# td-kwj-zp2023/webgpu-msm-bls12-377

Hardware: AMD Instinct MI355X
Metric: ms per 2^20 BLS12-377 G1 MSM (lower is better)
Workload: dtype u32 (29-bit limbs, 64-bit accumulate)

## Files before the change

webgpu-msm-bls12-377_amd/csrc/kernels/convert.hpp:

```cpp
#pragma once
#include "../curves.hpp"

namespace msm377 {
namespace {


__global__ void __launch_bounds__(256) k_clear_words(uint32_t* __restrict__ a, uint32_t na, uint32_t* __restrict__ b, uint32_t nb) {
  for (uint32_t i = threadIdx.x; i < na; i += 256) a[i] = 0;
  for (uint32_t i = threadIdx.x; i < nb; i += 256) b[i] = 0;
}

template <class CV>
__global__ void __launch_bounds__(256) k_convert_bases(const uint32_t* __restrict__ raw, uint32_t* __restrict__ bases, uint64_t n, int* __restrict__ err) {
  uint64_t i = (uint64_t)blockIdx.x * 256 + threadIdx.x;
  if (i >= n) return;
  uint32_t w[CV::RAW_WORDS];
  load_words16(raw + i * CV::RAW_WORDS, w, CV::RAW_WORDS / 4);
  uint32_t o[CV::REC_WORDS];
  if (CV::convert(w, o)) atomicOr(err, ERR_TE_CONVERT);
  uint4* dst = reinterpret_cast<uint4*>(bases + i * CV::REC_WORDS);
#pragma unroll
  for (int k = 0; k < (int)CV::REC_WORDS / 4; k++) dst[k] = make_uint4(o[4 * k], o[4 * k + 1], o[4 * k + 2], o[4 * k + 3]);
}


__device__ __forceinline__ void put13(uint32_t* w, const Fp::El& e) {
#pragma unroll
  for (int j = 0; j < 13; j++) w[j] = e.l[j];
}
__device__ __forceinline__ Fp::El get13(const uint32_t* w) {
  Fp::El e;
#pragma unroll
  for (int j = 0; j < 13; j++) e.l[j] = w[j];
  return e;
}
struct AffWireSource {
  const uint32_t* raw;
  __device__ __forceinline__ bool load(uint64_t i, Fp::El& n1, Fp::El& n2, Fp::El& z) const {
    using K = G1Consts;
    uint32_t w[24];
    load_words16(raw + i * 24, w, 6);
    const Fp::El xr = Fp::from_words<12>(w), yr = Fp::from_words<12>(w + 12);
    const Fp::El u = Fp::add_lz(Fp::mul_lz(xr, Fp::from_const(K::TE_SR)), Fp::from_const(K::TE_S));
    const Fp::El v = Fp::mul_lz(yr, Fp::from_const(K::TE_SR));
    const Fp::El cu = Fp::csub(Fp::norm(Fp::add_lz(Fp::mul_lz(xr, Fp::from_const(K::TE_CSR)), Fp::from_const(K::TE_CS))), K::MOD);
    const Fp::El up = Fp::add_lz(u, Fp::one());
    z = Fp::mul_lz(up, v);
    n1 = Fp::mul_lz(up, cu);
    n2 = Fp::norm(Fp::add_kp_sub_sub2(z, K::KP4W3, Fp::zero(), v));
    return Te377::is_zero_mod_p(z);
  }
};
struct AffDoublingSource {
  const uint32_t* prev;
  uint32_t bits;
  __device__ __forceinline__ bool load(uint64_t i, Fp::El& n1, Fp::El& n2, Fp::El& z) const {
    Te377::Ext p = Te377::from_base_affine(TeAffBase::load_base(prev, (uint32_t)i), false);
    bool bad = false;
#pragma unroll 1
    for (uint32_t k = 0; k < bits; k++) {
      p = Te377::add(p, p);
      bad |= Te377::is_bad(p);
    }
    n1 = Fp::canon(p.x);
    n2 = Fp::canon(p.y);
    z = Fp::canon(p.z);
    return bad;
  }
};
template <class SRC>
__global__ void __launch_bounds__(AFF_THREADS, 4) k_affine_up(SRC src, uint64_t n, uint32_t* __restrict__ stash,
                                                              uint32_t* __restrict__ trees, uint32_t* __restrict__ block_prod, uint32_t* __restrict__ host_flag, uint32_t* __restrict__ dev_count,
                                                              int* __restrict__ err, uint32_t prio) {
  if (prio) __builtin_amdgcn_s_setprio(3);
  using K = G1Consts;
  __shared__ uint32_t tree[2 * AFF_THREADS][13];
  const uint32_t tid = threadIdx.x, blk = blockIdx.x;
  const uint64_t base = (uint64_t)blk * AFF_BLOCK_POINTS + tid;
  bool bad = false;
  Fp::El c = Fp::one();
#pragma unroll 1
  for (uint32_t j = 0; j < AFF_K; j++) {
    const uint64_t i = base + (uint64_t)j * AFF_THREADS;
    if (i >= n) break;
    Fp::El n1, n2, z;
    if (src.load(i, n1, n2, z)) {
      bad = true;
      z = Fp::one();
    }
    uint32_t o[AFF_STASH_WORDS];
    put13(o, n1);
    put13(o + 13, n2);
    put13(o + 26, z);
    put13(o + 39, c);
    uint4* dst = reinterpret_cast<uint4*>(stash) + ((size_t)blk * AFF_K + j) * (AFF_STASH_WORDS / 4) * AFF_THREADS + tid;
#pragma unroll
    for (int k = 0; k < (int)AFF_STASH_WORDS / 4; k++) dst[(size_t)k * AFF_THREADS] = make_uint4(o[4 * k], o[4 * k + 1], o[4 * k + 2], o[4 * k + 3]);
    c = Fp::mul_lz(c, z);
  }
  if (bad) atomicOr(err, ERR_TE_CONVERT);
  put13(tree[AFF_THREADS + tid], c);
  for (uint32_t size = AFF_THREADS / 2; size >= 1; size >>= 1) {
    __syncthreads();
    if (tid < size) put13(tree[size + tid], Fp::mul_lz(get13(tree[2 * (size + tid)]), get13(tree[2 * (size + tid) + 1])));
  }
  __syncthreads();
  uint32_t* out = trees + (size_t)blk * (2 * AFF_THREADS * 13);
  const uint32_t* flat = &tree[0][0];
  for (uint32_t k = tid; k < 2 * AFF_THREADS * 13; k += AFF_THREADS) out[k] = flat[k];
  if (tid == 0) {
    const Fp::El root = Fp::mul(get13(tree[1]), Fp::from_const(K::TO64));
    uint32_t w[12];
    Fp::to_words<12>(root, w);
#pragma unroll
    for (int j = 0; j < 12; j++) block_prod[(size_t)blk * 12 + j] = w[j];
    __threadfence_system();
    if (atomicAdd(dev_count, 1u) == gridDim.x - 1) {
      *dev_count = 0;
      __threadfence_system();
      *reinterpret_cast<volatile uint32_t*>(host_flag) = gridDim.x;
    }
  }
}

__global__ void __launch_bounds__(AFF_THREADS, 2) k_affine_down(uint64_t n, const uint32_t* __restrict__ stash, const uint32_t* __restrict__ trees,
                                                                const uint32_t* __restrict__ block_inv, uint32_t* __restrict__ bases, uint32_t prio) {
  if (prio) __builtin_amdgcn_s_setprio(3);
  __shared__ uint32_t tree[2 * AFF_THREADS][13];
  const uint32_t tid = threadIdx.x, blk = blockIdx.x;
  const uint32_t* in = trees + (size_t)blk * (2 * AFF_THREADS * 13);
  uint32_t* flat = &tree[0][0];
  for (uint32_t k = tid; k < 2 * AFF_THREADS * 13; k += AFF_THREADS) flat[k] = in[k];
  __syncthreads();
  if (tid == 0) {
    uint32_t w[12];
#pragma unroll
    for (int j = 0; j < 12; j++) w[j] = block_inv[(size_t)blk * 12 + j];
    put13(tree[1], Fp::from_words<12>(w));
  }
  for (uint32_t size = 1; size < AFF_THREADS; size <<= 1) {
    __syncthreads();
    if (tid < size) {
      const uint32_t k = size + tid;
      const Fp::El inv_k = get13(tree[k]), a = get13(tree[2 * k]), b = get13(tree[2 * k + 1]);
      put13(tree[2 * k], Fp::mul_lz(inv_k, b));
      put13(tree[2 * k + 1], Fp::mul_lz(inv_k, a));
    }
  }
  __syncthreads();
  Fp::El inv = get13(tree[AFF_THREADS + tid]);
  const uint64_t base = (uint64_t)blk * AFF_BLOCK_POINTS + tid;
#pragma unroll 1
  for (int j = (int)AFF_K - 1; j >= 0; j--) {
    const uint64_t i = base + (uint64_t)j * AFF_THREADS;
    if (i >= n) continue;
    uint32_t w[AFF_STASH_WORDS];
    {
      const uint4* src = reinterpret_cast<const uint4*>(stash) + ((size_t)blk * AFF_K + j) * (AFF_STASH_WORDS / 4) * AFF_THREADS + tid;
#pragma unroll
      for (int k = 0; k < (int)AFF_STASH_WORDS / 4; k++) {
        const uint4 v = src[(size_t)k * AFF_THREADS];
        w[4 * k + 0] = v.x;
        w[4 * k + 1] = v.y;
        w[4 * k + 2] = v.z;
        w[4 * k + 3] = v.w;
      }
    }
    const Fp::El zi = Fp::mul_lz(inv, get13(w + 39));
    inv = Fp::mul_lz(inv, get13(w + 26));
    const Fp::El x = Fp::mul(get13(w), zi), y = Fp::mul(get13(w + 13), zi);
    const Fp::El ymx = Fp::sub(y, x), ypx = Fp::add(y, x), kt = Fp::mul_lz(Fp::mul_lz(x, y), Fp::from_const(G1Consts::TE_2D));
    uint32_t o[TeAffBase::REC_WORDS];
    put13(o, ymx);
    put13(o + 13, ypx);
    put13(o + 26, kt);
    o[39] = 0;
    uint4* dst = reinterpret_cast<uint4*>(bases + i * TeAffBase::REC_WORDS);
#pragma unroll
    for (int k = 0; k < (int)TeAffBase::REC_WORDS / 4; k++) dst[k] = make_uint4(o[4 * k], o[4 * k + 1], o[4 * k + 2], o[4 * k + 3]);
  }
}


__global__ void __launch_bounds__(256) k_convert_bases_glv(const uint32_t* __restrict__ raw, uint32_t* __restrict__ bases, uint64_t n) {
  uint64_t i = (uint64_t)blockIdx.x * 256 + threadIdx.x;
  if (i >= n) return;
  uint32_t w[24];
  load_words16(raw + i * 24, w, 6);
  const Fp::El x = Fp::to_mont(Fp::from_words<12>(w));
  const Fp::El y = Fp::to_mont(Fp::from_words<12>(w + 12));
  const Fp::El bx = Fp::mul(x, Fp::from_const(G1Consts::BETA));
  constexpr uint32_t REC_WORDS = G1Dev::REC_WORDS;
  uint32_t o[REC_WORDS];
#pragma unroll
  for (int j = 0; j < 13; j++) {
    o[j] = x.l[j];
    o[13 + j] = y.l[j];
  }
#pragma unroll
  for (int j = 26; j < 32; j++) o[j] = 0;
  uint4* dst = reinterpret_cast<uint4*>(bases + i * REC_WORDS);
#pragma unroll
  for (int k = 0; k < 8; k++) dst[k] = make_uint4(o[4 * k], o[4 * k + 1], o[4 * k + 2], o[4 * k + 3]);
#pragma unroll
  for (int j = 0; j < 13; j++) o[j] = bx.l[j];
  dst = reinterpret_cast<uint4*>(bases + (n + i) * REC_WORDS);
#pragma unroll
  for (int k = 0; k < 8; k++) dst[k] = make_uint4(o[4 * k], o[4 * k + 1], o[4 * k + 2], o[4 * k + 3]);
}


}
}
```

Measured before the change: 2.369.

## Prefetch stash rows and coalesce affine base stores through LDS in affine_down

Restructures the backward loop of k_affine_down so the next stash row is requested into registers before the current row's field arithmetic runs, hiding global load latency. Output records are staged in padded shared memory and then written to global memory in a block-wide coalesced pattern instead of each thread writing its own 160-byte record with strided uint4 stores. The tree buffer is aliased onto the new LDS staging array. This adds two barriers per row and more live registers for the prefetch buffer, which may reduce occupancy.

```diff
diff --git a/webgpu-msm-bls12-377_amd/csrc/kernels/convert.hpp b/webgpu-msm-bls12-377_amd/csrc/kernels/convert.hpp
--- a/webgpu-msm-bls12-377_amd/csrc/kernels/convert.hpp
+++ b/webgpu-msm-bls12-377_amd/csrc/kernels/convert.hpp
@@ -123,10 +123,20 @@
   }
 }
 
+constexpr uint32_t AFF_REC_PIECES = TeAffBase::REC_WORDS / 4, AFF_REC_PITCH = AFF_REC_PIECES + 1;
+constexpr uint32_t AFF_REC_LDS = AFF_THREADS * AFF_REC_PITCH;
+static_assert(AFF_REC_LDS >= 2 * AFF_THREADS * 13 / 4, "the tree fits the buffer");
+__device__ __forceinline__ uint32_t affine_rows(uint64_t first, uint64_t n) {
+  if (first >= n) return 0;
+  const uint64_t r = (n - first + AFF_THREADS - 1) / AFF_THREADS;
+  return r < AFF_K ? (uint32_t)r : AFF_K;
+}
+
 __global__ void __launch_bounds__(AFF_THREADS, 2) k_affine_down(uint64_t n, const uint32_t* __restrict__ stash, const uint32_t* __restrict__ trees,
                                                                 const uint32_t* __restrict__ block_inv, uint32_t* __restrict__ bases, uint32_t prio) {
   if (prio) __builtin_amdgcn_s_setprio(3);
-  __shared__ uint32_t tree[2 * AFF_THREADS][13];
+  __shared__ uint4 lds[AFF_REC_LDS];
+  uint32_t(*tree)[13] = reinterpret_cast<uint32_t(*)[13]>(lds);
   const uint32_t tid = threadIdx.x, blk = blockIdx.x;
   const uint32_t* in = trees + (size_t)blk * (2 * AFF_THREADS * 13);
   uint32_t* flat = &tree[0][0];
@@ -149,35 +159,52 @@
   }
   __syncthreads();
   Fp::El inv = get13(tree[AFF_THREADS + tid]);
-  const uint64_t base = (uint64_t)blk * AFF_BLOCK_POINTS + tid;
+  __syncthreads();
+  const uint64_t first = (uint64_t)blk * AFF_BLOCK_POINTS, base = first + tid;
+  const uint32_t rows = affine_rows(first, n);
+  constexpr uint32_t STASH_PIECES = AFF_STASH_WORDS / 4;
+  uint4 next[STASH_PIECES];
+  auto request = [&](uint32_t j) {
+    const uint4* src = reinterpret_cast<const uint4*>(stash) + ((size_t)blk * AFF_K + j) * STASH_PIECES * AFF_THREADS + tid;
+    const bool mine = base + (uint64_t)j * AFF_THREADS < n;
+#pragma unroll
+    for (uint32_t k = 0; k < STASH_PIECES; k++) next[k] = mine ? src[(size_t)k * AFF_THREADS] : make_uint4(0, 0, 0, 0);
+  };
+  if (rows) request(rows - 1);
 #pragma unroll 1
-  for (int j = (int)AFF_K - 1; j >= 0; j--) {
-    const uint64_t i = base + (uint64_t)j * AFF_THREADS;
-    if (i >= n) continue;
+  for (uint32_t j = rows; j-- > 0;) {
     uint32_t w[AFF_STASH_WORDS];
-    {
-      const uint4* src = reinterpret_cast<const uint4*>(stash) + ((size_t)blk * AFF_K + j) * (AFF_STASH_WORDS / 4) * AFF_THREADS + tid;
-#pragma unroll
-      for (int k = 0; k < (int)AFF_STASH_WORDS / 4; k++) {
-        const uint4 v = src[(size_t)k * AFF_THREADS];
-        w[4 * k + 0] = v.x;
-        w[4 * k + 1] = v.y;
-        w[4 * k + 2] = v.z;
-        w[4 * k + 3] = v.w;
-      }
-    }
-    const Fp::El zi = Fp::mul_lz(inv, get13(w + 39));
-    inv = Fp::mul_lz(inv, get13(w + 26));
-    const Fp::El x = Fp::mul(get13(w), zi), y = Fp::mul(get13(w + 13), zi);
-    const Fp::El ymx = Fp::sub(y, x), ypx = Fp::add(y, x), kt = Fp::mul_lz(Fp::mul_lz(x, y), Fp::from_const(G1Consts::TE_2D));
-    uint32_t o[TeAffBase::REC_WORDS];
-    put13(o, ymx);
-    put13(o + 13, ypx);
-    put13(o + 26, kt);
-    o[39] = 0;
-    uint4* dst = reinterpret_cast<uint4*>(bases + i * TeAffBase::REC_WORDS);
-#pragma unroll
-    for (int k = 0; k < (int)TeAffBase::REC_WORDS / 4; k++) dst[k] = make_uint4(o[4 * k], o[4 * k + 1], o[4 * k + 2], o[4 * k + 3]);
+#pragma unroll
+    for (uint32_t k = 0; k < STASH_PIECES; k++) {
+      w[4 * k + 0] = next[k].x;
+      w[4 * k + 1] = next[k].y;
+      w[4 * k + 2] = next[k].z;
+      w[4 * k + 3] = next[k].w;
+    }
+    if (j) request(j - 1);
+    const uint64_t p0 = first + (uint64_t)j * AFF_THREADS;
+    if (p0 + tid < n) {
+      const Fp::El zi = Fp::mul_lz(inv, get13(w + 39));
+      inv = Fp::mul_lz(inv, get13(w + 26));
+      const Fp::El x = Fp::mul(get13(w), zi), y = Fp::mul(get13(w + 13), zi);
+      const Fp::El ymx = Fp::sub(y, x), ypx = Fp::add(y, x), kt = Fp::mul_lz(Fp::mul_lz(x, y), Fp::from_const(G1Consts::TE_2D));
+      uint32_t o[TeAffBase::REC_WORDS];
+      put13(o, ymx);
+      put13(o + 13, ypx);
+      put13(o + 26, kt);
+      o[39] = 0;
+#pragma unroll
+      for (uint32_t k = 0; k < AFF_REC_PIECES; k++) lds[tid * AFF_REC_PITCH + k] = make_uint4(o[4 * k], o[4 * k + 1], o[4 * k + 2], o[4 * k + 3]);
+    }
+    __syncthreads();
+    const uint32_t have = (uint32_t)(n - p0 < AFF_THREADS ? n - p0 : AFF_THREADS) * AFF_REC_PIECES;
+    uint4* row = reinterpret_cast<uint4*>(bases) + p0 * AFF_REC_PIECES;
+#pragma unroll
+    for (uint32_t k = 0; k < AFF_REC_PIECES; k++) {
+      const uint32_t g = tid + k * AFF_THREADS;
+      if (g < have) row[g] = lds[(g / AFF_REC_PIECES) * AFF_REC_PITCH + g % AFF_REC_PIECES];
+    }
+    __syncthreads();
   }
 }
 
```

Measured after the change: 2.417. 1.02x slower.
